# jenndrei/BayHunter

Hardware: AMD Instinct MI355X
Metric: forward-model+logL evals/sec (batched 10-layer models) (higher is better)
Workload: dtype f64

## Files before the change

bayhunter_amd/csrc/chain_kernel.hip:

```cpp
#include "../../include/bh_engine.h"
#include "bh_device.h"
#ifndef BH_CHAIN_ABSENT
#define BH_CHAIN_ABSENT 0
#endif
#ifndef BH_CHAIN_PRIORS
#define BH_CHAIN_PRIORS 0
#endif
#ifndef BH_CHAIN_RECORD
#define BH_CHAIN_RECORD 0
#endif
#if BH_CHAIN_RECORD
#include "../../include/bh_engine_chain_record.h"
#define BH_RECORD_KPARAM , bh_chain_record store, int due, int due_step
#else
#define BH_RECORD_KPARAM
#endif
#if BH_CHAIN_PRIORS
#include "../../include/bh_engine_sites_priors.h"
#define ST pr
#define BH_NLO(i) pr.nb[(i) * pr.stride]
#define BH_NHI(i) pr.nb[(2 * BH_MAX_TARGETS + (i)) * pr.stride]
#define BH_NOISE_FREE(i) (BH_NLO(i) != BH_NHI(i) && ((absent >> ((i) >> 1)) & 1u) == 0u)
#define BH_PRIOR_OK (!pr.bad)
#define BH_SITE_PARAM , unsigned absent, const Prior &pr
#define BH_SITE_ARG(c) , (absent_of != nullptr ? (unsigned)absent_of[c] : 0u), pr
#define BH_SITE_KPARAM , const uint8_t *absent_of, const bh_chain_prior *priors, int NP, const int32_t *prior_of
#define BH_ACCEPT_KPARAM , const bh_chain_prior *priors, int NP, const int32_t *prior_of
#elif BH_CHAIN_ABSENT
#include "../../include/bh_engine_sites_missing.h"
#define ST cfg
#define BH_NLO(i) cfg.noise_lo[i]
#define BH_NHI(i) cfg.noise_hi[i]
#define BH_NOISE_FREE(i) (cfg.noise_lo[i] != cfg.noise_hi[i] && ((absent >> ((i) >> 1)) & 1u) == 0u)
#define BH_PRIOR_OK true
#define BH_SITE_PARAM , unsigned absent
#define BH_SITE_ARG(c) , (unsigned)absent_of[c]
#define BH_SITE_KPARAM , const uint8_t *absent_of
#else
#define ST cfg
#define BH_NLO(i) cfg.noise_lo[i]
#define BH_NHI(i) cfg.noise_hi[i]
#define BH_NOISE_FREE(i) (cfg.noise_lo[i] != cfg.noise_hi[i])
#define BH_PRIOR_OK true
#define BH_SITE_PARAM
#define BH_SITE_ARG(c)
#define BH_SITE_KPARAM
#define BH_ACCEPT_KPARAM
#endif

namespace {

struct Philox {
    uint32_t k0, k1;
    __device__ void round(uint32_t c[4])
    {
        const uint32_t M0 = 0xD2511F53u, M1 = 0xCD9E8D57u;
        const uint64_t p0 = (uint64_t)M0 * c[0], p1 = (uint64_t)M1 * c[2];
        const uint32_t hi0 = (uint32_t)(p0 >> 32), lo0 = (uint32_t)p0, hi1 = (uint32_t)(p1 >> 32), lo1 = (uint32_t)p1;
        const uint32_t n0 = hi1 ^ c[1] ^ k0, n1 = lo1, n2 = hi0 ^ c[3] ^ k1, n3 = lo0;
        c[0] = n0; c[1] = n1; c[2] = n2; c[3] = n3;
        k0 += 0x9E3779B9u;
        k1 += 0xBB67AE85u;
    }
    __device__ void gen(uint64_t seed, uint32_t a, uint32_t b, uint32_t cc, uint32_t out[4])
    {
        k0 = (uint32_t)seed;
        k1 = (uint32_t)(seed >> 32);
        uint32_t c[4] = {a, b, cc, 0u};
        for (int i = 0; i < 10; ++i) round(c);
        out[0] = c[0]; out[1] = c[1]; out[2] = c[2]; out[3] = c[3];
    }
};

__device__ __forceinline__ double u01(uint32_t hi, uint32_t lo)
{
    return (double)((((uint64_t)hi << 32) | lo) >> 11) * (1.0 / 9007199254740992.0);
}

#if !BH_CHAIN_RECORD
struct Draws {
    double u_move, u_index, u_z, u_accept, u_noise, normal;
};

__device__ Draws get_draws(const bh_chain_config &cfg, const bh_chain_state &S, int c, int C, int iiter, int k)
{
    Draws d;
    if (S.inject != nullptr) {
        const double *in = S.inject + (size_t)k * 6 * C;
        d.u_move = in[0 * (size_t)C + c]; d.u_index = in[1 * (size_t)C + c];
        d.u_z = in[2 * (size_t)C + c]; d.u_accept = in[3 * (size_t)C + c];
        d.u_noise = in[4 * (size_t)C + c]; d.normal = in[5 * (size_t)C + c];
        return d;
    }
    Philox ph;
    uint32_t r[4], q[4], t[4], n[4];
    const uint32_t gc = (uint32_t)(cfg.chain_offset + (int64_t)c);
    ph.gen(cfg.seed, gc, (uint32_t)iiter, 0u, r);
    ph.gen(cfg.seed, gc, (uint32_t)iiter, 1u, q);
    ph.gen(cfg.seed, gc, (uint32_t)iiter, 2u, t);
    ph.gen(cfg.seed, gc, (uint32_t)iiter, 3u, n);
    d.u_move = u01(r[0], r[1]); d.u_index = u01(r[2], r[3]);
    d.u_z = u01(q[0], q[1]); d.u_accept = u01(q[2], q[3]);
    d.u_noise = u01(t[0], t[1]);
    const double a = 1.0 - u01(n[0], n[1]);
    const double bq = u01(n[2], n[3]);
    d.normal = sqrt(-2.0 * log(a)) * cospi(2.0 * bq);
    return d;
}
#endif

#if !BH_CHAIN_ABSENT
__device__ double get_accept_draw(const bh_chain_config &cfg, const bh_chain_state &S, int c, int C, int iiter, int k)
{
    if (S.inject != nullptr) return S.inject[(size_t)k * 6 * C + 3 * (size_t)C + c];
    Philox ph;
    uint32_t q[4];
    ph.gen(cfg.seed, (uint32_t)(cfg.chain_offset + (int64_t)c), (uint32_t)iiter, 1u, q);
    return u01(q[2], q[3]);
}
#endif

enum { MV_VS = 0, MV_Z = 1, MV_BIRTH = 2, MV_DEATH = 3, MV_NOISE = 4, MV_VPVS = 5 };
__device__ __forceinline__ int par_index(int mv) { return mv <= 1 ? mv : (mv <= 3 ? 2 : mv - 1); }

struct Params {
    int n;
    double vpvs;
    double *vs, *z, *noise, *h;
};
#if BH_CHAIN_PRIORS
struct Prior {
    int layermin, layermax;
    double vsmin, vsmax, zmin, zmax, thickmin, lvz, hvz, vpvsmin, vpvsmax, mantle_vs, mantle_vpvs;
    const double *nb;
    int stride;
    bool bad;
};
__device__ __forceinline__ void fetch_prior(Prior &pr, const bh_chain_prior *priors, int NP, int k, double *nb, int stride, int first,
                                            int step)
{
    pr.nb = nb;
    pr.stride = stride;
    pr.bad = k < 0 || k >= NP;
    if (pr.bad) {
        pr.layermin = pr.layermax = 0;
        pr.vsmin = pr.vsmax = pr.zmin = pr.zmax = pr.thickmin = pr.vpvsmin = pr.vpvsmax = pr.mantle_vpvs = 0.0;
        pr.lvz = pr.hvz = pr.mantle_vs = -1.0;
        for (int i = first; i < 4 * BH_MAX_TARGETS; i += step) nb[i * stride] = 0.0;
        return;
    }
    const bh_chain_prior *__restrict__ r = priors + k;
    pr.layermin = r->layermin; pr.layermax = r->layermax;
    pr.vsmin = r->vsmin; pr.vsmax = r->vsmax; pr.zmin = r->zmin; pr.zmax = r->zmax;
    pr.thickmin = r->thickmin; pr.lvz = r->lvz; pr.hvz = r->hvz;
    pr.vpvsmin = r->vpvsmin; pr.vpvsmax = r->vpvsmax; pr.mantle_vs = r->mantle_vs; pr.mantle_vpvs = r->mantle_vpvs;
    for (int i = first; i < 4 * BH_MAX_TARGETS; i += step)
        nb[i * stride] = i < 2 * BH_MAX_TARGETS ? r->noise_lo[i] : r->noise_hi[i - 2 * BH_MAX_TARGETS];
}
struct AcceptPrior {
    double vsmin, vsmax, acc_lo, acc_hi;
};
#endif
__host__ __device__ inline int node_rec_doubles(int nt, int ML) { return 3 + 2 * nt + 3 * (ML + 1); }

#if !BH_CHAIN_RECORD
__device__ void load_base(const bh_chain_state &S, int C, size_t ldp, int nt, int ML, int c, int from_node, Params &P,
                          const double *lds_from = nullptr)
{
    if (from_node >= 0 && lds_from != nullptr) {
        const double *__restrict__ src = lds_from;
        double *__restrict__ pn = P.noise, *__restrict__ pv = P.vs, *__restrict__ pz = P.z;
        P.n = (int)src[0];
        P.vpvs = src[2];
        for (int i = 0; i < 2 * nt; ++i) pn[i] = src[3 + i];
        const double *__restrict__ fv = src + 3 + 2 * nt, *__restrict__ fz = fv + (ML + 1);
        const int n = P.n;
#pragma unroll 4
        for (int i = 0; i < n; ++i) {
            pv[i] = fv[i];
            pz[i] = fz[i];
        }
        return;
    }
    if (from_node < 0) {
        P.n = S.n[c];
        for (int i = 0; i < P.n; ++i) {
            P.vs[i] = S.vs[(size_t)i * C + c];
            P.z[i] = S.z[(size_t)i * C + c];
        }
        P.vpvs = S.vpvs[c];
        for (int i = 0; i < 2 * nt; ++i) P.noise[i] = S.noise[(size_t)i * C + c];
    } else {
        const size_t col = (size_t)from_node * C + c;
        P.n = S.pn[col];
        for (int i = 0; i < P.n; ++i) {
            P.vs[i] = S.pvs[(size_t)i * ldp + col];
            P.z[i] = S.pz[(size_t)i * ldp + col];
        }
        P.vpvs = S.pvpvs[col];
        for (int i = 0; i < 2 * nt; ++i) P.noise[i] = S.pnoise[col * 2 * nt + i];
    }
}

__device__ __forceinline__ void layer_thicknesses(const Params &P, double *h_)
{
    const double *__restrict__ z = P.z;
    double *__restrict__ h = h_;
    const int n = P.n;
    double prev = 0.0, zi = n >= 1 ? z[0] : 0.0;
#pragma unroll 4
    for (int i = 0; i + 1 < n; ++i) {
        const double zn = z[i + 1];
        const double zd = (zi + zn) / 2.;
        h[i] = zd - prev;
        prev = zd;
        zi = zn;
    }
    if (n >= 1) h[n - 1] = 0.0;
}

__device__ __forceinline__ int nearest_nucleus(const double *__restrict__ z, int n, double zb)
{
    int near = 0;
    double best = fabs(z[0] - zb);
#pragma unroll 4
    for (int i = 1; i < n; ++i) {
        const double di = fabs(z[i] - zb);
        if (di < best) {
            best = di;
            near = i;
        }
    }
    return near;
}

__device__ __forceinline__ void propose_node(const bh_chain_config &cfg, const bh_chain_state &S, int C, size_t ldp, int c, int iiter,
                                             int from_node, int node, Params &P, const double *lds_from, bool *valid_out, const Draws &d BH_SITE_PARAM)
{
    const int ML = cfg.maxlayers, nt = cfg.nt;
    int nnoise = 0;
    for (int i = 0; i < 2 * nt; ++i) nnoise += BH_NOISE_FREE(i);
    const bool vpvs_free = ST.vpvsmin != ST.vpvsmax;
    const bool early = (double)iiter < (-(double)cfg.iter_burnin + (double)cfg.iterations * 0.01);
    int moves[6], nm = 0;
    moves[nm++] = MV_VS;
    moves[nm++] = MV_Z;
    if (!early) {
        moves[nm++] = MV_BIRTH;
        moves[nm++] = MV_DEATH;
    }
    if (nnoise > 0) moves[nm++] = MV_NOISE;
    if (vpvs_free) moves[nm++] = MV_VPVS;
    int mi = (int)(d.u_move * nm);
    if (mi >= nm) mi = nm - 1;
    const int mv = moves[mi];

    load_base(S, C, ldp, nt, ML, c, from_node, P, lds_from);
    double *vs = P.vs, *z = P.z, *noise = P.noise;
    int n = P.n;
    double vpvs = P.vpvs;
    double dvs2 = 0.0;
    bool valid = BH_PRIOR_OK;
    if (mv == MV_VS) {
        int ind = (int)(d.u_index * n);
        if (ind >= n) ind = n - 1;
        vs[ind] = vs[ind] + d.normal * S.propdist[0 * (size_t)C + c];
    } else if (mv == MV_Z) {
        int ind = (int)(d.u_index * n);
        if (ind >= n) ind = n - 1;
        z[ind] = z[ind] + d.normal * S.propdist[1 * (size_t)C + c];
    } else if (mv == MV_BIRTH) {
        const double zb = ST.zmin + d.u_z * (ST.zmax - ST.zmin);
        const int near = nearest_nucleus(z, n, zb);
        const double vb = vs[near] + d.normal * S.propdist[2 * (size_t)C + c];
        dvs2 = (vb - vs[near]) * (vb - vs[near]);
        if (n >= ML) valid = false;
        else {
            vs[n] = vb;
            z[n] = zb;
            n += 1;
        }
    } else if (mv == MV_DEATH) {
        int ind = (int)(d.u_index * n);
        if (ind >= n) ind = n - 1;
        const double zb = z[ind], vb = vs[ind];
        for (int i = ind; i + 1 < n; ++i) {
            vs[i] = vs[i + 1];
            z[i] = z[i + 1];
        }
        n -= 1;
        if (n < 1) valid = false;
        else {
            const int near = nearest_nucleus(z, n, zb);
            dvs2 = (vs[near] - vb) * (vs[near] - vb);
        }
    } else if (mv == MV_NOISE) {
        int pick = (int)(d.u_noise * nnoise);
        if (pick >= nnoise) pick = nnoise - 1;
        int idx = 0;
        for (int i = 0, seen = 0; i < 2 * nt; ++i)
            if (BH_NOISE_FREE(i)) {
                if (seen == pick) idx = i;
                ++seen;
            }
        noise[idx] = noise[idx] + d.normal * S.propdist[3 * (size_t)C + c];
        for (int i = 0; i < 2 * nt; ++i)
            if (BH_NOISE_FREE(i) && (noise[i] < BH_NLO(i) || noise[i] > BH_NHI(i))) valid = false;
    } else {
        vpvs = vpvs + d.normal * S.propdist[4 * (size_t)C + c];
        if (vpvs < ST.vpvsmin || vpvs > ST.vpvsmax) valid = false;
    }
    double ztop = n > 0 ? z[0] : 0.0;
    for (int i = 1; i < n; ++i) {
        const double zi = z[i];
        if (!(ztop > zi)) {
            ztop = zi;
            continue;
        }
        const double vi = vs[i];
        int j = i - 1;
        while (j >= 0 && z[j] > zi) {
            z[j + 1] = z[j];
            vs[j + 1] = vs[j];
            --j;
        }
        z[j + 1] = zi;
        vs[j + 1] = vi;
    }
    P.n = n;
    P.vpvs = vpvs;
    double *h = P.h;
    layer_thicknesses(P, h);
    if (valid && (mv <= MV_DEATH)) {
        const int layermodel = n - 1;
        if (!(layermodel >= ST.layermin && layermodel <= ST.layermax)) valid = false;
        const double *__restrict__ rh = h, *__restrict__ rv = vs;
        double zc = 0.0, vi = n > 0 ? rv[0] : 0.0;
        bool ok = true;
#pragma unroll 4
        for (int i = 0; i < n; ++i) {
            const double hi = rh[i];
            const double vn = (i + 1 < n) ? rv[i + 1] : 0.0;
            if (i < n - 1 && hi < ST.thickmin) ok = false;
            if (vi < ST.vsmin || vi > ST.vsmax) ok = false;
            zc += hi;
            if (zc < ST.zmin || zc > ST.zmax) ok = false;
            if (i + 1 < n) {
                if (ST.lvz >= 0.0 && !(vn - vi * (1 - ST.lvz) > 0)) ok = false;
                if (ST.hvz >= 0.0 && !(vi * (1 + ST.hvz) - vn > 0)) ok = false;
            }
            vi = vn;
        }
        valid = valid && ok;
    }
    const size_t col = (size_t)node * C + c;
    S.move[col] = mv;
    S.valid[col] = valid ? 1 : 0;
    S.dvs2[col] = dvs2;
    if (!valid) {
        load_base(S, C, ldp, nt, ML, c, from_node, P, lds_from);
        layer_thicknesses(P, h);
        n = P.n;
        vpvs = P.vpvs;
    }
    P.n = n;
    P.vpvs = vpvs;
    *valid_out = valid;
    S.pn[col] = n;
    S.pvpvs[col] = vpvs;
    for (int i = 0; i < 2 * nt; ++i) S.pnoise[col * 2 * nt + i] = noise[i];
    {
        const double *__restrict__ rv = vs, *__restrict__ rz = z, *__restrict__ rh = h;
        bool deep = false;
#pragma unroll 4
        for (int i = 0; i < n; ++i) {
            const double vi = rv[i], zi = rz[i], hi = rh[i];
            if (ST.mantle_vs > 0.0 && vi >= ST.mantle_vs) deep = true;
            S.pvs[(size_t)i * ldp + col] = vi;
            S.pz[(size_t)i * ldp + col] = zi;
            S.lay_h[(size_t)i * ldp + col] = hi;
            S.lay_vs[(size_t)i * ldp + col] = vi;
            const double vpi = vi * (deep ? ST.mantle_vpvs : vpvs);
            S.lay_vp[(size_t)i * ldp + col] = vpi;
            if (S.lay_rho != nullptr) S.lay_rho[(size_t)i * ldp + col] = vpi * 0.32 + 0.77;
        }
    }
    S.lay_n[col] = n;
}

__global__ void chain_propose_kernel(bh_chain_config cfg, bh_chain_state S, int C, int iiter BH_SITE_KPARAM)
{
    const int c = blockIdx.x * blockDim.x + threadIdx.x;
    if (c >= C) return;
    double vs[BH_CHAIN_MAXLAYERS + 1], z[BH_CHAIN_MAXLAYERS + 1], h[BH_CHAIN_MAXLAYERS + 1], noise[2 * BH_MAX_TARGETS];
    Params P;
    P.vs = vs; P.z = z; P.h = h; P.noise = noise;
#if BH_CHAIN_PRIORS
    __shared__ double nb[4 * BH_MAX_TARGETS * 64];
    Prior pr;
    fetch_prior(pr, priors, NP, prior_of[c], nb + threadIdx.x, 64, 0, 1);
#endif
    bool valid;
    propose_node(cfg, S, C, (size_t)C, c, iiter, -1, 0, P, nullptr, &valid, get_draws(cfg, S, c, C, iiter, 0) BH_SITE_ARG(c));
}

__global__ __launch_bounds__(64) void chain_propose_window_kernel(bh_chain_config cfg, bh_chain_state S, int C, size_t ldp,
                                                                   int iiter, int depth BH_SITE_KPARAM)
{
    extern __shared__ __align__(16) double tree[];
    const int T = 1 << (depth - 1);
    const int per_wg = 64 / T;
    const int N = (1 << depth) - 1;
    const int slot = (int)threadIdx.x / T;
    const int c = blockIdx.x * per_wg + slot;
    const int p = (int)threadIdx.x % T;
    const int nt = cfg.nt, ML = cfg.maxlayers;
    const int RS = node_rec_doubles(nt, ML) | 1;
    double *mine = tree + (size_t)slot * N * RS;
#if BH_CHAIN_PRIORS
    double *nbw = tree + (size_t)per_wg * N * RS;
    Prior pr;
    {
        fetch_prior(pr, priors, NP, c < C ? prior_of[c] : -1, nbw + slot, per_wg, p, T);
        __builtin_amdgcn_fence(__ATOMIC_RELEASE, "wavefront");
        __builtin_amdgcn_wave_barrier();
        __builtin_amdgcn_fence(__ATOMIC_ACQUIRE, "wavefront");
    }
#endif
    Draws mydraws = {0.0, 0.0, 0.0, 0.0, 0.0, 0.0};
    if (c < C && p < depth) mydraws = get_draws(cfg, S, c, C, iiter + p, p);
    for (int k = 0; k < depth; ++k) {
        const int srcl = slot * T + k;
        Draws d;
        d.u_move = __shfl(mydraws.u_move, srcl); d.u_index = __shfl(mydraws.u_index, srcl);
        d.u_z = __shfl(mydraws.u_z, srcl); d.u_accept = __shfl(mydraws.u_accept, srcl);
        d.u_noise = __shfl(mydraws.u_noise, srcl); d.normal = __shfl(mydraws.normal, srcl);
        if (c < C && p < (1 << k)) {
            const int node = (1 << k) - 1 + p;
            int from = -1;
            for (int j = node; j > 0; j = (j - 1) >> 1) {
                const int parent = (j - 1) >> 1;
                if ((j & 1) == 0 && mine[(size_t)parent * RS + 1] != 0.0) {
                    from = parent;
                    break;
                }
            }
            double *rec = mine + (size_t)node * RS;
            Params P;
            P.noise = rec + 3;
            P.vs = rec + 3 + 2 * nt;
            P.z = P.vs + (ML + 1);
            P.h = P.z + (ML + 1);
            bool valid;
            propose_node(cfg, S, C, ldp, c, iiter + k, from, node, P, from >= 0 ? mine + (size_t)from * RS : nullptr, &valid, d BH_SITE_ARG(c));
            rec[0] = (double)P.n;
            rec[1] = valid ? 1.0 : 0.0;
            rec[2] = P.vpvs;
        }
        __builtin_amdgcn_fence(__ATOMIC_RELEASE, "wavefront");
        __builtin_amdgcn_wave_barrier();
        __builtin_amdgcn_fence(__ATOMIC_ACQUIRE, "wavefront");
    }
}
#endif

#if !BH_CHAIN_ABSENT && !BH_CHAIN_RECORD
__global__ void chain_accept_kernel(bh_chain_config cfg, bh_chain_state S, int C, size_t ldp, int iiter, int depth,
                                    const double *logL, const double *misfits BH_ACCEPT_KPARAM)
{
    const int c = blockIdx.x * blockDim.x + threadIdx.x;
    if (c >= C) return;
#if BH_CHAIN_PRIORS
    const int rec = prior_of[c];
    if (rec < 0 || rec >= NP) return;
    const AcceptPrior pr = {priors[rec].vsmin, priors[rec].vsmax, priors[rec].acc_lo, priors[rec].acc_hi};
#endif
    const int nt = cfg.nt;
    int node = 0, last = -1;
    double cur = S.like[c];
    const double beta = S.beta ? S.beta[c] : 1.0;
    for (int k = 0; k < depth; ++k) {
        const size_t col = (size_t)node * C + c;
        bool accepted = false;
        if (S.valid[col]) {
            const double u_accept = get_accept_draw(cfg, S, c, C, iiter + k, k);
            const int mv = S.move[col];
            const int pi = par_index(mv);
            S.proposed[pi * (size_t)C + c] += 1.0;
            const double like = logL[col];
            const double dl = (S.beta ? beta * (like - cur) : like - cur);
            double alpha;
            if (mv == MV_BIRTH || mv == MV_DEATH) {
                const double theta = S.propdist[2 * (size_t)C + c];
                const double dv = ST.vsmax - ST.vsmin;
                const double Bt = S.dvs2[col] / (2. * (theta * theta));
                if (mv == MV_BIRTH) alpha = log((theta * sqrt(2 * M_PI)) / dv) + Bt + dl;
                else alpha = log(dv / (theta * sqrt(2 * M_PI))) - Bt + dl;
            } else {
                alpha = dl;
            }
            if (log(u_accept) < alpha) {
                accepted = true;
                last = node;
                cur = like;
                S.accepted[pi * (size_t)C + c] += 1.0;
                S.naccepted[c] += 1;
            }
            if ((iiter + k) % 1000 == 0) {
                bool all = true;
                for (int i = 0; i < 5; ++i) all = all && (S.proposed[i * (size_t)C + c] != 0.0);
                if (all)
                    for (int i = 0; i < 5; ++i) {
                        const double rate = S.accepted[i * (size_t)C + c] / S.proposed[i * (size_t)C + c] * 100;
                        double pd = S.propdist[i * (size_t)C + c];
                        if (rate < ST.acc_lo) {
                            pd = pd * 0.95;
                            if (pd < 0.001) pd = 0.001;
                        } else if (rate > ST.acc_hi) {
                            pd = pd * 1.05;
                        }
                        S.propdist[i * (size_t)C + c] = pd;
                    }
            }
        }
        node = 2 * node + (accepted ? 2 : 1);
    }
    if (last >= 0) {
        const size_t col = (size_t)last * C + c;
        const int n = S.pn[col];
        S.n[c] = n;
        for (int i = 0; i < n; ++i) {
            S.vs[(size_t)i * C + c] = S.pvs[(size_t)i * ldp + col];
            S.z[(size_t)i * C + c] = S.pz[(size_t)i * ldp + col];
        }
        for (int i = n; i < cfg.maxlayers; ++i) {
            S.vs[(size_t)i * C + c] = 0.0;
            S.z[(size_t)i * C + c] = 0.0;
        }
        S.vpvs[c] = S.pvpvs[col];
        for (int i = 0; i < 2 * nt; ++i) S.noise[(size_t)i * C + c] = S.pnoise[col * 2 * nt + i];
        S.like[c] = cur;
        for (int i = 0; i <= nt; ++i) S.misfits[(size_t)i * C + c] = misfits[col * (nt + 1) + i];
    }
}
// ... 120 lines not shown
    if (lane < 5) {
        S.proposed[lane * (size_t)C + c] = prop;
        S.accepted[lane * (size_t)C + c] = acc;
    }
    if (lane == 0) S.naccepted[c] = nacc;
    if (last >= 0) {
        const size_t col = (size_t)last * C + c;
        const int n = S.pn[col];
        for (int i = lane; i < cfg.maxlayers; i += 64) {
            S.vs[(size_t)i * C + c] = i < n ? S.pvs[(size_t)i * ldp + col] : 0.0;
            S.z[(size_t)i * C + c] = i < n ? S.pz[(size_t)i * ldp + col] : 0.0;
        }
        for (int i = lane; i < 2 * nt; i += 64) S.noise[(size_t)i * C + c] = S.pnoise[col * 2 * nt + i];
        for (int i = lane; i <= nt; i += 64) S.misfits[(size_t)i * C + c] = misfits[col * (nt + 1) + i];
        if (lane == 0) {
            S.n[c] = n;
            S.vpvs[c] = S.pvpvs[col];
            S.like[c] = cur;
        }
    }
}

#endif

}

extern "C" {

#if BH_CHAIN_RECORD
#if BH_CHAIN_PRIORS
int bh_chain_accept_window_priors_record(void *stream, const bh_chain_config *cfg, const bh_chain_state *state, int C, int iiter,
                                         int depth, ptrdiff_t ld, const double *logL, const double *misfits,
                                         const bh_chain_prior *priors, int P, const int32_t *prior_of, const bh_chain_record *rec)
#else
int bh_chain_accept_window_record(void *stream, const bh_chain_config *cfg, const bh_chain_state *state, int C, int iiter,
                                  int depth, ptrdiff_t ld, const double *logL, const double *misfits, const bh_chain_record *rec)
#endif
{
    if (!cfg || !state || C < 0 || !logL || !misfits) return BH_EINVAL;
    if (cfg->maxlayers < 0 || cfg->maxlayers > BH_CHAIN_MAXLAYERS || cfg->nt < 0 || cfg->nt > BH_MAX_TARGETS) return BH_EINVAL;
    if (depth < 1 || depth > BH_CHAIN_MAXDEPTH || ld < (ptrdiff_t)C * ((1 << depth) - 1)) return BH_EINVAL;
#if BH_CHAIN_PRIORS
    if (!priors || !prior_of || P < 1) return BH_EINVAL;
#endif
    for (int k = 0; k + 1 < depth; ++k)
        if ((iiter + k) % 1000 == 0) return BH_EINVAL;
    if (!rec || !rec->models || !rec->likes || !rec->vpvs || !rec->misfits || !rec->noise) return BH_EINVAL;
    if (rec->thinning < 1 || rec->row0 < 0) return BH_EINVAL;
    const int64_t res = (((int64_t)iiter % rec->thinning) + rec->thinning) % rec->thinning;
    const int64_t first = res == 0 ? 0 : rec->thinning - res;
    const int64_t m = first >= depth ? 0 : 1 + ((int64_t)depth - 1 - first) / rec->thinning;
    if (rec->row0 > rec->rows - m) return BH_EINVAL;
    if (C == 0) return BH_OK;
    const int due = (int)(first < depth ? first : depth);
    const int due_step = (int)(rec->thinning <= BH_CHAIN_MAXDEPTH ? rec->thinning : BH_CHAIN_MAXDEPTH + 1);
#if BH_CHAIN_PRIORS
    hipLaunchKernelGGL(chain_accept_window_kernel, dim3(C), dim3(64), 0, (hipStream_t)stream, *cfg, *state, C, (size_t)ld, iiter, depth,
                       logL, misfits, priors, P, prior_of, *rec, due, due_step);
#else
    hipLaunchKernelGGL(chain_accept_window_kernel, dim3(C), dim3(64), 0, (hipStream_t)stream, *cfg, *state, C, (size_t)ld, iiter, depth,
                       logL, misfits, *rec, due, due_step);
#endif
    return hipGetLastError() == hipSuccess ? BH_OK : BH_EHIP;
}

#elif BH_CHAIN_PRIORS
static int window_args_ok(const bh_chain_config *cfg, const bh_chain_state *state, int C, int iiter, int depth, ptrdiff_t ld,
                          const bh_chain_prior *priors, int P, const int32_t *prior_of)
{
    if (!cfg || !state || C < 0 || cfg->maxlayers > BH_CHAIN_MAXLAYERS || cfg->nt > BH_MAX_TARGETS) return 0;
    if (depth < 1 || depth > BH_CHAIN_MAXDEPTH || ld < (ptrdiff_t)C * ((1 << depth) - 1)) return 0;
    if (!priors || !prior_of || P < 1) return 0;
    for (int k = 0; k + 1 < depth; ++k)
        if ((iiter + k) % 1000 == 0) return 0;
    return 1;
}

int bh_chain_propose_window_priors(void *stream, const bh_chain_config *cfg, const bh_chain_state *state, int C, int iiter,
                                   int depth, ptrdiff_t ld, const bh_chain_prior *priors, int P, const int32_t *prior_of,
                                   const uint8_t *absent)
{
    if (!window_args_ok(cfg, state, C, iiter, depth, ld, priors, P, prior_of)) return BH_EINVAL;
    if (C == 0) return BH_OK;
    if (depth == 1 && ld == C) {
        hipLaunchKernelGGL(chain_propose_kernel, dim3((C + 63) / 64), dim3(64), 0, (hipStream_t)stream, *cfg, *state, C, iiter, absent,
                           priors, P, prior_of);
    } else {
        const int per_wg = 64 >> (depth - 1);
        const size_t lds = ((size_t)per_wg * ((1 << depth) - 1) * (node_rec_doubles(cfg->nt, cfg->maxlayers) | 1) +
                            (size_t)per_wg * 4 * BH_MAX_TARGETS) * sizeof(double);
        if (lds > 160 * 1024) return BH_EUNSUPPORTED;
        if (lds > 64 * 1024) {
            static std::atomic<unsigned long long> big{0};
            const void *k[1] = {reinterpret_cast<const void *>(chain_propose_window_kernel)};
            if (!bh_allow_big_lds(&big, k, 1, 160 * 1024)) return BH_EHIP;
        }
        hipLaunchKernelGGL(chain_propose_window_kernel, dim3((C + per_wg - 1) / per_wg), dim3(64), lds, (hipStream_t)stream, *cfg,
                           *state, C, (size_t)ld, iiter, depth, absent, priors, P, prior_of);
    }
    return hipGetLastError() == hipSuccess ? BH_OK : BH_EHIP;
}

int bh_chain_propose_priors(void *stream, const bh_chain_config *cfg, const bh_chain_state *state, int C, int iiter,
                            const bh_chain_prior *priors, int P, const int32_t *prior_of, const uint8_t *absent)
{
    return bh_chain_propose_window_priors(stream, cfg, state, C, iiter, 1, C, priors, P, prior_of, absent);
}

int bh_chain_accept_window_priors(void *stream, const bh_chain_config *cfg, const bh_chain_state *state, int C, int iiter,
                                  int depth, ptrdiff_t ld, const double *logL, const double *misfits,
                                  const bh_chain_prior *priors, int P, const int32_t *prior_of)
{
    if (!window_args_ok(cfg, state, C, iiter, depth, ld, priors, P, prior_of) || !logL || !misfits) return BH_EINVAL;
    if (C == 0) return BH_OK;
    if (depth > 1)
        hipLaunchKernelGGL(chain_accept_window_kernel, dim3(C), dim3(64), 0, (hipStream_t)stream, *cfg, *state, C, (size_t)ld, iiter, depth,
                           logL, misfits, priors, P, prior_of);
    else
        hipLaunchKernelGGL(chain_accept_kernel, dim3((C + 63) / 64), dim3(64), 0, (hipStream_t)stream, *cfg, *state, C, (size_t)ld,
                           iiter, depth, logL, misfits, priors, P, prior_of);
    return hipGetLastError() == hipSuccess ? BH_OK : BH_EHIP;
}

int bh_chain_accept_priors(void *stream, const bh_chain_config *cfg, const bh_chain_state *state, int C, int iiter,
                           const double *logL, const double *misfits, const bh_chain_prior *priors, int P,
                           const int32_t *prior_of)
{
    return bh_chain_accept_window_priors(stream, cfg, state, C, iiter, 1, C, logL, misfits, priors, P, prior_of);
}

#else

#if BH_CHAIN_ABSENT
int bh_chain_propose_window_sites(void *stream, const bh_chain_config *cfg, const bh_chain_state *state, int C, int iiter,
                                  int depth, ptrdiff_t ld, const uint8_t *absent)
#else
int bh_chain_propose_window(void *stream, const bh_chain_config *cfg, const bh_chain_state *state, int C, int iiter,
                            int depth, ptrdiff_t ld)
#endif
{
#if BH_CHAIN_ABSENT
    if (!absent) return BH_EINVAL;
#define BH_ABSENT_LAUNCH , absent
#else
#define BH_ABSENT_LAUNCH
#endif
    if (!cfg || !state || C < 0 || cfg->maxlayers > BH_CHAIN_MAXLAYERS || cfg->nt > BH_MAX_TARGETS) return BH_EINVAL;
    if (depth < 1 || depth > BH_CHAIN_MAXDEPTH || ld < (ptrdiff_t)C * ((1 << depth) - 1)) return BH_EINVAL;
    for (int k = 0; k + 1 < depth; ++k)
        if ((iiter + k) % 1000 == 0) return BH_EINVAL;
    if (C == 0) return BH_OK;
    if (depth == 1 && ld == C) {
        hipLaunchKernelGGL(chain_propose_kernel, dim3((C + 63) / 64), dim3(64), 0, (hipStream_t)stream, *cfg, *state, C, iiter BH_ABSENT_LAUNCH);
    } else {
        const int per_wg = 64 >> (depth - 1);
        const size_t lds = (size_t)per_wg * ((1 << depth) - 1) * (node_rec_doubles(cfg->nt, cfg->maxlayers) | 1) * sizeof(double);
        if (lds > 160 * 1024) return BH_EUNSUPPORTED;
        if (lds > 64 * 1024) {
            static std::atomic<unsigned long long> big{0};
            const void *k[1] = {reinterpret_cast<const void *>(chain_propose_window_kernel)};
            if (!bh_allow_big_lds(&big, k, 1, 160 * 1024)) return BH_EHIP;
        }
        hipLaunchKernelGGL(chain_propose_window_kernel, dim3((C + per_wg - 1) / per_wg), dim3(64), lds, (hipStream_t)stream, *cfg,
                           *state, C, (size_t)ld, iiter, depth BH_ABSENT_LAUNCH);
    }
    return hipGetLastError() == hipSuccess ? BH_OK : BH_EHIP;
}
#undef BH_ABSENT_LAUNCH

#if BH_CHAIN_ABSENT
int bh_chain_propose_sites(void *stream, const bh_chain_config *cfg, const bh_chain_state *state, int C, int iiter, const uint8_t *absent)
{
    return bh_chain_propose_window_sites(stream, cfg, state, C, iiter, 1, C, absent);
}
#else

int bh_chain_accept_window(void *stream, const bh_chain_config *cfg, const bh_chain_state *state, int C, int iiter, int depth,
                           ptrdiff_t ld, const double *logL, const double *misfits)
{
    if (!cfg || !state || C < 0 || !logL || !misfits) return BH_EINVAL;
    if (depth < 1 || depth > BH_CHAIN_MAXDEPTH || ld < (ptrdiff_t)C * ((1 << depth) - 1)) return BH_EINVAL;
    for (int k = 0; k + 1 < depth; ++k)
        if ((iiter + k) % 1000 == 0) return BH_EINVAL;
    if (C == 0) return BH_OK;
    if (depth > 1)
        hipLaunchKernelGGL(chain_accept_window_kernel, dim3(C), dim3(64), 0, (hipStream_t)stream, *cfg, *state, C, (size_t)ld, iiter, depth,
                           logL, misfits);
    else
        hipLaunchKernelGGL(chain_accept_kernel, dim3((C + 63) / 64), dim3(64), 0, (hipStream_t)stream, *cfg, *state, C, (size_t)ld,
                           iiter, depth, logL, misfits);
    return hipGetLastError() == hipSuccess ? BH_OK : BH_EHIP;
}

int bh_chain_propose(void *stream, const bh_chain_config *cfg, const bh_chain_state *state, int C, int iiter)
{
    return bh_chain_propose_window(stream, cfg, state, C, iiter, 1, C);
}

int bh_chain_accept(void *stream, const bh_chain_config *cfg, const bh_chain_state *state, int C, int iiter,
                    const double *logL, const double *misfits)
{
    return bh_chain_accept_window(stream, cfg, state, C, iiter, 1, C, logL, misfits);
}

#endif

#endif

}
```

Baseline: 6.170 million.

## Parallelise chain proposal across lanes per chain with one workgroup per chain

Rewrites the MCMC proposal kernel so each chain gets its own workgroup, and each tree node is handled by a group of lanes rather than one thread. Nearest-nucleus search, layer sorting (rank-based instead of insertion sort), thickness and constraint checks, and noise checks become lane-parallel with ballots and shuffles. The base model, draws and proposal widths are staged in LDS once, and moves are expressed as virtual edits over the parent record instead of copied arrays. The separate depth-1 kernel path is dropped. This trades more threads and LDS per chain, plus extra barriers, for less serial per-thread work.

New measurement: 6.150 million. About the same (-0.3%).

```diff
diff --git a/bayhunter_amd/csrc/chain_kernel.hip b/bayhunter_amd/csrc/chain_kernel.hip
--- a/bayhunter_amd/csrc/chain_kernel.hip
+++ b/bayhunter_amd/csrc/chain_kernel.hip
@@ -22,28 +22,30 @@
 #define BH_NHI(i) pr.nb[(2 * BH_MAX_TARGETS + (i)) * pr.stride]
 #define BH_NOISE_FREE(i) (BH_NLO(i) != BH_NHI(i) && ((absent >> ((i) >> 1)) & 1u) == 0u)
 #define BH_PRIOR_OK (!pr.bad)
-#define BH_SITE_PARAM , unsigned absent, const Prior &pr
-#define BH_SITE_ARG(c) , (absent_of != nullptr ? (unsigned)absent_of[c] : 0u), pr
+#define BH_SITE_PARAM , const Prior &pr
+#define BH_SITE_ARG , pr
+#define BH_ABSENT_OF(c) (absent_of != nullptr ? (unsigned)absent_of[c] : 0u)
 #define BH_SITE_KPARAM , const uint8_t *absent_of, const bh_chain_prior *priors, int NP, const int32_t *prior_of
 #define BH_ACCEPT_KPARAM , const bh_chain_prior *priors, int NP, const int32_t *prior_of
 #elif BH_CHAIN_ABSENT
 #include "../../include/bh_engine_sites_missing.h"
 #define ST cfg
-#define BH_NLO(i) cfg.noise_lo[i]
-#define BH_NHI(i) cfg.noise_hi[i]
-#define BH_NOISE_FREE(i) (cfg.noise_lo[i] != cfg.noise_hi[i] && ((absent >> ((i) >> 1)) & 1u) == 0u)
+#define BH_NLO(i) nb[i]
+#define BH_NHI(i) nb[2 * BH_MAX_TARGETS + (i)]
+#define BH_NOISE_FREE(i) (BH_NLO(i) != BH_NHI(i) && ((absent >> ((i) >> 1)) & 1u) == 0u)
 #define BH_PRIOR_OK true
-#define BH_SITE_PARAM , unsigned absent
-#define BH_SITE_ARG(c) , (unsigned)absent_of[c]
+#define BH_SITE_PARAM , const double *nb
+#define BH_SITE_ARG , nb
+#define BH_ABSENT_OF(c) ((unsigned)absent_of[c])
 #define BH_SITE_KPARAM , const uint8_t *absent_of
 #else
 #define ST cfg
-#define BH_NLO(i) cfg.noise_lo[i]
-#define BH_NHI(i) cfg.noise_hi[i]
-#define BH_NOISE_FREE(i) (cfg.noise_lo[i] != cfg.noise_hi[i])
+#define BH_NLO(i) nb[i]
+#define BH_NHI(i) nb[2 * BH_MAX_TARGETS + (i)]
+#define BH_NOISE_FREE(i) (BH_NLO(i) != BH_NHI(i))
 #define BH_PRIOR_OK true
-#define BH_SITE_PARAM
-#define BH_SITE_ARG(c)
+#define BH_SITE_PARAM , const double *nb
+#define BH_SITE_ARG , nb
 #define BH_SITE_KPARAM
 #define BH_ACCEPT_KPARAM
 #endif
@@ -123,11 +125,6 @@
 enum { MV_VS = 0, MV_Z = 1, MV_BIRTH = 2, MV_DEATH = 3, MV_NOISE = 4, MV_VPVS = 5 };
 __device__ __forceinline__ int par_index(int mv) { return mv <= 1 ? mv : (mv <= 3 ? 2 : mv - 1); }
 
-struct Params {
-    int n;
-    double vpvs;
-    double *vs, *z, *noise, *h;
-};
 #if BH_CHAIN_PRIORS
 struct Prior {
     int layermin, layermax;
@@ -162,220 +159,277 @@
 };
 #endif
 __host__ __device__ inline int node_rec_doubles(int nt, int ML) { return 3 + 2 * nt + 3 * (ML + 1); }
+#ifndef BH_PROPOSE_LANES
+#define BH_PROPOSE_LANES 32
+#endif
+#ifndef BH_PROPOSE_MAXTHREADS
+#define BH_PROPOSE_MAXTHREADS 512
+#endif
+__host__ __device__ inline int propose_threads(int depth)
+{
+    const int t = BH_PROPOSE_LANES << (depth - 1);
+    return t < 64 ? 64 : (t > BH_PROPOSE_MAXTHREADS ? BH_PROPOSE_MAXTHREADS : t);
+}
+enum { PROPOSE_HDR = 6 * BH_CHAIN_MAXDEPTH + 5 + 1 };
+__host__ __device__ inline size_t propose_lds_doubles(int nt, int ML, int depth)
+{
+    return ((size_t)1 << depth) * (size_t)(node_rec_doubles(nt, ML) | 1) + PROPOSE_HDR + 4 * BH_MAX_TARGETS + (((size_t)1 << depth) + 1) / 2;
+}
 
 #if !BH_CHAIN_RECORD
-__device__ void load_base(const bh_chain_state &S, int C, size_t ldp, int nt, int ML, int c, int from_node, Params &P,
-                          const double *lds_from = nullptr)
-{
-    if (from_node >= 0 && lds_from != nullptr) {
-        const double *__restrict__ src = lds_from;
-        double *__restrict__ pn = P.noise, *__restrict__ pv = P.vs, *__restrict__ pz = P.z;
-        P.n = (int)src[0];
-        P.vpvs = src[2];
-        for (int i = 0; i < 2 * nt; ++i) pn[i] = src[3 + i];
-        const double *__restrict__ fv = src + 3 + 2 * nt, *__restrict__ fz = fv + (ML + 1);
-        const int n = P.n;
-#pragma unroll 4
-        for (int i = 0; i < n; ++i) {
-            pv[i] = fv[i];
-            pz[i] = fz[i];
-        }
-        return;
-    }
-    if (from_node < 0) {
-        P.n = S.n[c];
-        for (int i = 0; i < P.n; ++i) {
-            P.vs[i] = S.vs[(size_t)i * C + c];
-            P.z[i] = S.z[(size_t)i * C + c];
-        }
-        P.vpvs = S.vpvs[c];
-        for (int i = 0; i < 2 * nt; ++i) P.noise[i] = S.noise[(size_t)i * C + c];
-    } else {
-        const size_t col = (size_t)from_node * C + c;
-        P.n = S.pn[col];
-        for (int i = 0; i < P.n; ++i) {
-            P.vs[i] = S.pvs[(size_t)i * ldp + col];
-            P.z[i] = S.pz[(size_t)i * ldp + col];
-        }
-        P.vpvs = S.pvpvs[col];
-        for (int i = 0; i < 2 * nt; ++i) P.noise[i] = S.pnoise[col * 2 * nt + i];
-    }
-}
-
-__device__ __forceinline__ void layer_thicknesses(const Params &P, double *h_)
-{
-    const double *__restrict__ z = P.z;
-    double *__restrict__ h = h_;
-    const int n = P.n;
-    double prev = 0.0, zi = n >= 1 ? z[0] : 0.0;
-#pragma unroll 4
-    for (int i = 0; i + 1 < n; ++i) {
-        const double zn = z[i + 1];
-        const double zd = (zi + zn) / 2.;
-        h[i] = zd - prev;
-        prev = zd;
-        zi = zn;
-    }
-    if (n >= 1) h[n - 1] = 0.0;
-}
-
-__device__ __forceinline__ int nearest_nucleus(const double *__restrict__ z, int n, double zb)
-{
-    int near = 0;
-    double best = fabs(z[0] - zb);
-#pragma unroll 4
-    for (int i = 1; i < n; ++i) {
-        const double di = fabs(z[i] - zb);
-        if (di < best) {
-            best = di;
-            near = i;
-        }
-    }
-    return near;
+struct Lanes {
+    int g, W, first;
+    unsigned long long mask;
+};
+__device__ __forceinline__ unsigned long long group_ballot(const Lanes &G, bool p) { return (__ballot(p) >> G.first) & G.mask; }
+__device__ __forceinline__ void group_sync()
+{
+    __builtin_amdgcn_fence(__ATOMIC_RELEASE, "wavefront");
+    __builtin_amdgcn_wave_barrier();
+    __builtin_amdgcn_fence(__ATOMIC_ACQUIRE, "wavefront");
+}
+
+struct Moved {
+    const double *sv, *sz;
+    int del, rv, rz;
+    double newv, newz;
+    __device__ __forceinline__ double z(int j) const
+    {
+        const double v = sz[j + (j >= del ? 1 : 0)];
+        return j == rz ? newz : v;
+    }
+    __device__ __forceinline__ double vs(int j) const
+    {
+        const double v = sv[j + (j >= del ? 1 : 0)];
+        return j == rv ? newv : v;
+    }
+};
+
+__device__ __forceinline__ int nearest_nucleus(const Lanes &G, const Moved &M, int n, double zb)
+{
+    double best = __builtin_huge_val();
+    int near = 0x7fffffff;
+    for (int i0 = 0; i0 < n; i0 += G.W) {
+        const int i = i0 + G.g;
+        if (i < n) {
+            const double di = fabs(M.z(i) - zb);
+            if (i == 0 || di < best) {
+                best = di;
+                near = i;
+            }
+        }
+    }
+    for (int off = G.W >> 1; off >= 1; off >>= 1) {
+        const double bo = __shfl_xor(best, off);
+        const int no = __shfl_xor(near, off);
+        if (bo < best || (bo == best && no < near)) {
+            best = bo;
+            near = no;
+        }
+    }
+    near = __shfl(near, G.first);
+    return near < 0 ? 0 : (near < n ? near : (n > 0 ? n - 1 : 0));
+}
+
+__device__ __forceinline__ bool layers_of(const Lanes &G, int n, const double *ov, const double *oz, double *oh, bool check,
+                                          double thickmin, double vsmin, double vsmax, double lvz, double hvz)
+{
+    bool anybad = false;
+    for (int i0 = 0; i0 < n; i0 += G.W) {
+        const int i = i0 + G.g;
+        bool bad = false;
+        if (i < n) {
+            const double zi = oz[i];
+            const double prev = i > 0 ? (oz[i - 1] + zi) / 2. : 0.0;
+            double hi = 0.0;
+            if (i + 1 < n) {
+                const double zd = (zi + oz[i + 1]) / 2.;
+                hi = zd - prev;
+            }
+            oh[i] = hi;
+            if (check) {
+                const double vi = ov[i];
+                if (i < n - 1 && hi < thickmin) bad = true;
+                if (vi < vsmin || vi > vsmax) bad = true;
+                if (i + 1 < n) {
+                    const double vn = ov[i + 1];
+                    if (lvz >= 0.0 && !(vn - vi * (1 - lvz) > 0)) bad = true;
+                    if (hvz >= 0.0 && !(vi * (1 + hvz) - vn > 0)) bad = true;
+                }
+            }
+        }
+        if (check && group_ballot(G, bad) != 0ull) anybad = true;
+    }
+    return anybad;
 }
 
 __device__ __forceinline__ void propose_node(const bh_chain_config &cfg, const bh_chain_state &S, int C, size_t ldp, int c, int iiter,
-                                             int from_node, int node, Params &P, const double *lds_from, bool *valid_out, const Draws &d BH_SITE_PARAM)
-{
-    const int ML = cfg.maxlayers, nt = cfg.nt;
-    int nnoise = 0;
-    for (int i = 0; i < 2 * nt; ++i) nnoise += BH_NOISE_FREE(i);
+                                             int node, const double *src, double *rec, const Lanes &G, const Draws &d, const double *pd,
+                                             unsigned nfree BH_SITE_PARAM)
+{
+    const int ML = cfg.maxlayers, nt = cfg.nt, g = G.g, W = G.W;
+    const int nnoise = __popc(nfree);
     const bool vpvs_free = ST.vpvsmin != ST.vpvsmax;
     const bool early = (double)iiter < (-(double)cfg.iter_burnin + (double)cfg.iterations * 0.01);
-    int moves[6], nm = 0;
-    moves[nm++] = MV_VS;
-    moves[nm++] = MV_Z;
-    if (!early) {
-        moves[nm++] = MV_BIRTH;
-        moves[nm++] = MV_DEATH;
-    }
-    if (nnoise > 0) moves[nm++] = MV_NOISE;
-    if (vpvs_free) moves[nm++] = MV_VPVS;
+    const int nm = 2 + (early ? 0 : 2) + (nnoise > 0 ? 1 : 0) + (vpvs_free ? 1 : 0);
     int mi = (int)(d.u_move * nm);
     if (mi >= nm) mi = nm - 1;
-    const int mv = moves[mi];
-
-    load_base(S, C, ldp, nt, ML, c, from_node, P, lds_from);
-    double *vs = P.vs, *z = P.z, *noise = P.noise;
-    int n = P.n;
-    double vpvs = P.vpvs;
-    double dvs2 = 0.0;
+    int mv;
+    if (mi < 2) mv = mi;
+    else if (!early && mi < 4) mv = mi;
+    else mv = (nnoise > 0 && mi == (early ? 2 : 4)) ? MV_NOISE : MV_VPVS;
+
+    const double *sn = src + 3, *sv = src + 3 + 2 * nt, *sz = sv + (ML + 1);
+    double *on = rec + 3, *ov = rec + 3 + 2 * nt, *oz = ov + (ML + 1), *oh = oz + (ML + 1);
+    const int n0 = (int)src[0];
+    const double vpvs0 = src[2];
+    int n = n0, noise_at = -1;
+    double vpvs = vpvs0, dvs2 = 0.0;
     bool valid = BH_PRIOR_OK;
-    if (mv == MV_VS) {
-        int ind = (int)(d.u_index * n);
-        if (ind >= n) ind = n - 1;
-        vs[ind] = vs[ind] + d.normal * S.propdist[0 * (size_t)C + c];
-    } else if (mv == MV_Z) {
-        int ind = (int)(d.u_index * n);
-        if (ind >= n) ind = n - 1;
-        z[ind] = z[ind] + d.normal * S.propdist[1 * (size_t)C + c];
-    } else if (mv == MV_BIRTH) {
-        const double zb = ST.zmin + d.u_z * (ST.zmax - ST.zmin);
-        const int near = nearest_nucleus(z, n, zb);
-        const double vb = vs[near] + d.normal * S.propdist[2 * (size_t)C + c];
-        dvs2 = (vb - vs[near]) * (vb - vs[near]);
-        if (n >= ML) valid = false;
+    Moved M = {sv, sz, 0x7fffffff, -1, -1, 0.0, 0.0};
+    if (mv <= MV_Z) {
+        int ind = (int)(d.u_index * n0);
+        if (ind >= n0) ind = n0 - 1;
+        if (ind < 0) ind = 0;
+        if (mv == MV_VS) {
+            M.newv = sv[ind] + d.normal * pd[0];
+            M.rv = ind;
+        } else {
+            M.newz = sz[ind] + d.normal * pd[1];
+            M.rz = ind;
+        }
+    } else if (mv <= MV_DEATH) {
+        double zb, vb = 0.0;
+        int among = n0;
+        if (mv == MV_BIRTH) zb = ST.zmin + d.u_z * (ST.zmax - ST.zmin);
         else {
-            vs[n] = vb;
-            z[n] = zb;
-            n += 1;
-        }
-    } else if (mv == MV_DEATH) {
-        int ind = (int)(d.u_index * n);
-        if (ind >= n) ind = n - 1;
-        const double zb = z[ind], vb = vs[ind];
-        for (int i = ind; i + 1 < n; ++i) {
-            vs[i] = vs[i + 1];
-            z[i] = z[i + 1];
-        }
-        n -= 1;
-        if (n < 1) valid = false;
-        else {
-            const int near = nearest_nucleus(z, n, zb);
-            dvs2 = (vs[near] - vb) * (vs[near] - vb);
+            int ind = (int)(d.u_index * n0);
+            if (ind >= n0) ind = n0 - 1;
+            if (ind < 0) ind = 0;
+            zb = sz[ind];
+            vb = sv[ind];
+            M.del = ind;
+            n = n0 - 1;
+            if (n < 1) {
+                valid = false;
+                n = 0;
+            }
+            among = n;
+        }
+        if (among >= 1) {
+            const int near = nearest_nucleus(G, M, among, zb);
+            const double vn = M.vs(near);
+            if (mv == MV_BIRTH) {
+                vb = vn + d.normal * pd[2];
+                dvs2 = (vb - vn) * (vb - vn);
+            } else {
+                dvs2 = (vn - vb) * (vn - vb);
+            }
+        }
+        if (mv == MV_BIRTH) {
+            if (n0 >= ML) valid = false;
+            else {
+                M.rv = M.rz = n0;
+                M.newv = vb;
+                M.newz = zb;
+                n = n0 + 1;
+            }
         }
     } else if (mv == MV_NOISE) {
         int pick = (int)(d.u_noise * nnoise);
         if (pick >= nnoise) pick = nnoise - 1;
-        int idx = 0;
-        for (int i = 0, seen = 0; i < 2 * nt; ++i)
-            if (BH_NOISE_FREE(i)) {
-                if (seen == pick) idx = i;
-                ++seen;
-            }
-        noise[idx] = noise[idx] + d.normal * S.propdist[3 * (size_t)C + c];
-        for (int i = 0; i < 2 * nt; ++i)
-            if (BH_NOISE_FREE(i) && (noise[i] < BH_NLO(i) || noise[i] > BH_NHI(i))) valid = false;
+        unsigned b = nfree;
+        for (int k = 0; k < pick; ++k) b &= b - 1u;
+        noise_at = b != 0u ? __ffs(b) - 1 : 0;
     } else {
-        vpvs = vpvs + d.normal * S.propdist[4 * (size_t)C + c];
+        vpvs = vpvs0 + d.normal * pd[4];
         if (vpvs < ST.vpvsmin || vpvs > ST.vpvsmax) valid = false;
     }
-    double ztop = n > 0 ? z[0] : 0.0;
-    for (int i = 1; i < n; ++i) {
-        const double zi = z[i];
-        if (!(ztop > zi)) {
-            ztop = zi;
-            continue;
-        }
-        const double vi = vs[i];
-        int j = i - 1;
-        while (j >= 0 && z[j] > zi) {
-            z[j + 1] = z[j];
-            vs[j + 1] = vs[j];
-            --j;
-        }
-        z[j + 1] = zi;
-        vs[j + 1] = vi;
-    }
-    P.n = n;
-    P.vpvs = vpvs;
-    double *h = P.h;
-    layer_thicknesses(P, h);
-    if (valid && (mv <= MV_DEATH)) {
+    for (int i0 = 0; i0 < 2 * nt; i0 += W) {
+        const int i = i0 + g;
+        bool bad = false;
+        if (i < 2 * nt) {
+            double v = sn[i];
+            if (i == noise_at) v = v + d.normal * pd[3];
+            on[i] = v;
+            if (mv == MV_NOISE && ((nfree >> i) & 1u) != 0u && (v < BH_NLO(i) || v > BH_NHI(i))) bad = true;
+        }
+        if (group_ballot(G, bad) != 0ull) valid = false;
+    }
+    for (int i0 = 0; i0 < n; i0 += W) {
+        const int i = i0 + g;
+        if (i < n) oh[i] = M.z(i);
+    }
+    group_sync();
+    for (int i0 = 0; i0 < n; i0 += W) {
+        const int i = i0 + g;
+        if (i < n) {
+            const double zi = oh[i], vi = M.vs(i);
+            int r = 0;
+#pragma unroll 8
+            for (int j = 0; j < n; ++j) {
+                const double zj = oh[j];
+                r += (zj < zi || (zj == zi && j < i)) ? 1 : 0;
+            }
+            oz[r] = zi;
+            ov[r] = vi;
+        }
+    }
+    group_sync();
+    const bool check = valid && mv <= MV_DEATH;
+    if (check) {
         const int layermodel = n - 1;
         if (!(layermodel >= ST.layermin && layermodel <= ST.layermax)) valid = false;
-        const double *__restrict__ rh = h, *__restrict__ rv = vs;
-        double zc = 0.0, vi = n > 0 ? rv[0] : 0.0;
+    }
+    if (layers_of(G, n, ov, oz, oh, check, ST.thickmin, ST.vsmin, ST.vsmax, ST.lvz, ST.hvz)) valid = false;
+    group_sync();
+    if (check) {
+        double zc = 0.0;
         bool ok = true;
-#pragma unroll 4
+#pragma unroll 8
         for (int i = 0; i < n; ++i) {
-            const double hi = rh[i];
-            const double vn = (i + 1 < n) ? rv[i + 1] : 0.0;
-            if (i < n - 1 && hi < ST.thickmin) ok = false;
-            if (vi < ST.vsmin || vi > ST.vsmax) ok = false;
-            zc += hi;
+            zc += oh[i];
             if (zc < ST.zmin || zc > ST.zmax) ok = false;
-            if (i + 1 < n) {
-                if (ST.lvz >= 0.0 && !(vn - vi * (1 - ST.lvz) > 0)) ok = false;
-                if (ST.hvz >= 0.0 && !(vi * (1 + ST.hvz) - vn > 0)) ok = false;
-            }
-            vi = vn;
-        }
-        valid = valid && ok;
+        }
+        if (!ok) valid = false;
+    }
+    if (!valid) {
+        n = n0;
+        vpvs = vpvs0;
+        for (int i0 = 0; i0 < n; i0 += W) {
+            const int i = i0 + g;
+            if (i < n) {
+                oz[i] = sz[i];
+                ov[i] = sv[i];
+            }
+        }
+        for (int i = g; i < 2 * nt; i += W) on[i] = sn[i];
+        group_sync();
+        layers_of(G, n, ov, oz, oh, false, 0.0, 0.0, 0.0, 0.0, 0.0);
+        group_sync();
     }
     const size_t col = (size_t)node * C + c;
-    S.move[col] = mv;
-    S.valid[col] = valid ? 1 : 0;
-    S.dvs2[col] = dvs2;
-    if (!valid) {
-        load_base(S, C, ldp, nt, ML, c, from_node, P, lds_from);
-        layer_thicknesses(P, h);
-        n = P.n;
-        vpvs = P.vpvs;
-    }
-    P.n = n;
-    P.vpvs = vpvs;
-    *valid_out = valid;
-    S.pn[col] = n;
-    S.pvpvs[col] = vpvs;
-    for (int i = 0; i < 2 * nt; ++i) S.pnoise[col * 2 * nt + i] = noise[i];
-    {
-        const double *__restrict__ rv = vs, *__restrict__ rz = z, *__restrict__ rh = h;
-        bool deep = false;
-#pragma unroll 4
-        for (int i = 0; i < n; ++i) {
-            const double vi = rv[i], zi = rz[i], hi = rh[i];
-            if (ST.mantle_vs > 0.0 && vi >= ST.mantle_vs) deep = true;
+    if (g == 0) {
+        rec[0] = (double)n;
+        rec[1] = valid ? 1.0 : 0.0;
+        rec[2] = vpvs;
+        S.move[col] = mv;
+        S.valid[col] = valid ? 1 : 0;
+        S.dvs2[col] = dvs2;
+        S.pn[col] = n;
+        S.pvpvs[col] = vpvs;
+        S.lay_n[col] = n;
+    }
+    for (int i = g; i < 2 * nt; i += W) S.pnoise[col * 2 * nt + i] = on[i];
+    bool deep_before = false;
+    for (int i0 = 0; i0 < n; i0 += W) {
+        const int i = i0 + g;
+        double vi = 0.0;
+        if (i < n) vi = ov[i];
+        const unsigned long long m = group_ballot(G, i < n && ST.mantle_vs > 0.0 && vi >= ST.mantle_vs);
+        const bool deep = deep_before || (m & ((2ull << g) - 1ull)) != 0ull;
+        if (i < n) {
+            const double zi = oz[i], hi = oh[i];
             S.pvs[(size_t)i * ldp + col] = vi;
             S.pz[(size_t)i * ldp + col] = zi;
             S.lay_h[(size_t)i * ldp + col] = hi;
@@ -384,82 +438,82 @@
             S.lay_vp[(size_t)i * ldp + col] = vpi;
             if (S.lay_rho != nullptr) S.lay_rho[(size_t)i * ldp + col] = vpi * 0.32 + 0.77;
         }
-    }
-    S.lay_n[col] = n;
-}
-
-__global__ void chain_propose_kernel(bh_chain_config cfg, bh_chain_state S, int C, int iiter BH_SITE_KPARAM)
-{
-    const int c = blockIdx.x * blockDim.x + threadIdx.x;
-    if (c >= C) return;
-    double vs[BH_CHAIN_MAXLAYERS + 1], z[BH_CHAIN_MAXLAYERS + 1], h[BH_CHAIN_MAXLAYERS + 1], noise[2 * BH_MAX_TARGETS];
-    Params P;
-    P.vs = vs; P.z = z; P.h = h; P.noise = noise;
-#if BH_CHAIN_PRIORS
-    __shared__ double nb[4 * BH_MAX_TARGETS * 64];
-    Prior pr;
-    fetch_prior(pr, priors, NP, prior_of[c], nb + threadIdx.x, 64, 0, 1);
-#endif
-    bool valid;
-    propose_node(cfg, S, C, (size_t)C, c, iiter, -1, 0, P, nullptr, &valid, get_draws(cfg, S, c, C, iiter, 0) BH_SITE_ARG(c));
-}
-
-__global__ __launch_bounds__(64) void chain_propose_window_kernel(bh_chain_config cfg, bh_chain_state S, int C, size_t ldp,
-                                                                   int iiter, int depth BH_SITE_KPARAM)
+        deep_before = deep_before || m != 0ull;
+    }
+}
+
+__global__ __launch_bounds__(BH_PROPOSE_MAXTHREADS) void chain_propose_window_kernel(bh_chain_config cfg, bh_chain_state S, int C, size_t ldp,
+                                                                     int iiter, int depth BH_SITE_KPARAM)
 {
     extern __shared__ __align__(16) double tree[];
-    const int T = 1 << (depth - 1);
-    const int per_wg = 64 / T;
+    const int tid = (int)threadIdx.x, NT = (int)blockDim.x;
+    const int c = (int)blockIdx.x;
     const int N = (1 << depth) - 1;
-    const int slot = (int)threadIdx.x / T;
-    const int c = blockIdx.x * per_wg + slot;
-    const int p = (int)threadIdx.x % T;
     const int nt = cfg.nt, ML = cfg.maxlayers;
     const int RS = node_rec_doubles(nt, ML) | 1;
-    double *mine = tree + (size_t)slot * N * RS;
+    double *hdr = tree + (size_t)(N + 1) * RS;
+    double *pd = hdr + 6 * BH_CHAIN_MAXDEPTH;
 #if BH_CHAIN_PRIORS
-    double *nbw = tree + (size_t)per_wg * N * RS;
     Prior pr;
+    fetch_prior(pr, priors, NP, prior_of[c], hdr + PROPOSE_HDR, 1, tid, NT);
+#else
+    double *nb = hdr + PROPOSE_HDR;
+    for (int i = tid; i < 2 * BH_MAX_TARGETS; i += NT) {
+        nb[i] = cfg.noise_lo[i];
+        nb[2 * BH_MAX_TARGETS + i] = cfg.noise_hi[i];
+    }
+#endif
     {
-        fetch_prior(pr, priors, NP, c < C ? prior_of[c] : -1, nbw + slot, per_wg, p, T);
-        __builtin_amdgcn_fence(__ATOMIC_RELEASE, "wavefront");
-        __builtin_amdgcn_wave_barrier();
-        __builtin_amdgcn_fence(__ATOMIC_ACQUIRE, "wavefront");
-    }
-#endif
-    Draws mydraws = {0.0, 0.0, 0.0, 0.0, 0.0, 0.0};
-    if (c < C && p < depth) mydraws = get_draws(cfg, S, c, C, iiter + p, p);
+        int n = S.n[c];
+        n = n < 0 ? 0 : (n > ML ? ML : n);
+        double *r0v = tree + 3 + 2 * nt, *r0z = r0v + (ML + 1);
+        for (int i = tid; i < n; i += NT) {
+            r0v[i] = S.vs[(size_t)i * C + c];
+            r0z[i] = S.z[(size_t)i * C + c];
+        }
+        for (int i = tid; i < 2 * nt; i += NT) tree[3 + i] = S.noise[(size_t)i * C + c];
+        if (tid == 0) {
+            tree[0] = (double)n;
+            tree[1] = 1.0;
+            tree[2] = S.vpvs[c];
+        }
+        if (tid < 5) pd[tid] = S.propdist[(size_t)tid * C + c];
+    }
+    if (tid < depth) {
+        const Draws w = get_draws(cfg, S, c, C, iiter + tid, tid);
+        double *o = hdr + 6 * tid;
+        o[0] = w.u_move; o[1] = w.u_index; o[2] = w.u_z; o[3] = w.u_accept; o[4] = w.u_noise; o[5] = w.normal;
+    }
+    __syncthreads();
+#if BH_CHAIN_PRIORS || BH_CHAIN_ABSENT
+    const unsigned absent = BH_ABSENT_OF(c);
+#endif
+    const unsigned nfree = (unsigned)__ballot((tid & 63) < 2 * nt && BH_NOISE_FREE(tid & 63));
+    int *base_of = reinterpret_cast<int *>(hdr + PROPOSE_HDR + 4 * BH_MAX_TARGETS);
+    int lg = 6;
+    while ((1 << lg) < NT) ++lg;
     for (int k = 0; k < depth; ++k) {
-        const int srcl = slot * T + k;
-        Draws d;
-        d.u_move = __shfl(mydraws.u_move, srcl); d.u_index = __shfl(mydraws.u_index, srcl);
-        d.u_z = __shfl(mydraws.u_z, srcl); d.u_accept = __shfl(mydraws.u_accept, srcl);
-        d.u_noise = __shfl(mydraws.u_noise, srcl); d.normal = __shfl(mydraws.normal, srcl);
-        if (c < C && p < (1 << k)) {
+        const int per = NT >> k;
+        const int p = tid >> (lg - k), g = tid & (per - 1);
+        if (g < 64) {
+            Lanes G;
+            G.g = g;
+            G.W = per < 64 ? per : 64;
+            G.first = (tid & 63) & ~(G.W - 1);
+            G.mask = G.W == 64 ? ~0ull : ((1ull << G.W) - 1ull);
+            const double *dk = hdr + 6 * k;
+            const Draws d = {dk[0], dk[1], dk[2], dk[3], dk[4], dk[5]};
             const int node = (1 << k) - 1 + p;
             int from = -1;
-            for (int j = node; j > 0; j = (j - 1) >> 1) {
-                const int parent = (j - 1) >> 1;
-                if ((j & 1) == 0 && mine[(size_t)parent * RS + 1] != 0.0) {
-                    from = parent;
-                    break;
-                }
-            }
-            double *rec = mine + (size_t)node * RS;
-            Params P;
-            P.noise = rec + 3;
-            P.vs = rec + 3 + 2 * nt;
-            P.z = P.vs + (ML + 1);
-            P.h = P.z + (ML + 1);
-            bool valid;
-            propose_node(cfg, S, C, ldp, c, iiter + k, from, node, P, from >= 0 ? mine + (size_t)from * RS : nullptr, &valid, d BH_SITE_ARG(c));
-            rec[0] = (double)P.n;
-            rec[1] = valid ? 1.0 : 0.0;
-            rec[2] = P.vpvs;
-        }
-        __builtin_amdgcn_fence(__ATOMIC_RELEASE, "wavefront");
-        __builtin_amdgcn_wave_barrier();
-        __builtin_amdgcn_fence(__ATOMIC_ACQUIRE, "wavefront");
+            if (node > 0) {
+                const int parent = (node - 1) >> 1;
+                from = ((node & 1) == 0 && tree[(size_t)(parent + 1) * RS + 1] != 0.0) ? parent : base_of[parent];
+            }
+            if (g == 0) base_of[node] = from;
+            propose_node(cfg, S, C, ldp, c, iiter + k, node, tree + (size_t)(from + 1) * RS, tree + (size_t)(node + 1) * RS, G, d, pd,
+                         nfree BH_SITE_ARG);
+        }
+        __syncthreads();
     }
 }
 #endif
@@ -746,20 +800,15 @@
 {
     if (!window_args_ok(cfg, state, C, iiter, depth, ld, priors, P, prior_of)) return BH_EINVAL;
     if (C == 0) return BH_OK;
-    if (depth == 1 && ld == C) {
-        hipLaunchKernelGGL(chain_propose_kernel, dim3((C + 63) / 64), dim3(64), 0, (hipStream_t)stream, *cfg, *state, C, iiter, absent,
-                           priors, P, prior_of);
-    } else {
-        const int per_wg = 64 >> (depth - 1);
-        const size_t lds = ((size_t)per_wg * ((1 << depth) - 1) * (node_rec_doubles(cfg->nt, cfg->maxlayers) | 1) +
-                            (size_t)per_wg * 4 * BH_MAX_TARGETS) * sizeof(double);
+    {
+        const size_t lds = propose_lds_doubles(cfg->nt, cfg->maxlayers, depth) * sizeof(double);
         if (lds > 160 * 1024) return BH_EUNSUPPORTED;
         if (lds > 64 * 1024) {
             static std::atomic<unsigned long long> big{0};
             const void *k[1] = {reinterpret_cast<const void *>(chain_propose_window_kernel)};
             if (!bh_allow_big_lds(&big, k, 1, 160 * 1024)) return BH_EHIP;
         }
-        hipLaunchKernelGGL(chain_propose_window_kernel, dim3((C + per_wg - 1) / per_wg), dim3(64), lds, (hipStream_t)stream, *cfg,
+        hipLaunchKernelGGL(chain_propose_window_kernel, dim3(C), dim3(propose_threads(depth)), lds, (hipStream_t)stream, *cfg,
                            *state, C, (size_t)ld, iiter, depth, absent, priors, P, prior_of);
     }
     return hipGetLastError() == hipSuccess ? BH_OK : BH_EHIP;
@@ -814,18 +863,15 @@
     for (int k = 0; k + 1 < depth; ++k)
         if ((iiter + k) % 1000 == 0) return BH_EINVAL;
     if (C == 0) return BH_OK;
-    if (depth == 1 && ld == C) {
-        hipLaunchKernelGGL(chain_propose_kernel, dim3((C + 63) / 64), dim3(64), 0, (hipStream_t)stream, *cfg, *state, C, iiter BH_ABSENT_LAUNCH);
-    } else {
-        const int per_wg = 64 >> (depth - 1);
-        const size_t lds = (size_t)per_wg * ((1 << depth) - 1) * (node_rec_doubles(cfg->nt, cfg->maxlayers) | 1) * sizeof(double);
+    {
+        const size_t lds = propose_lds_doubles(cfg->nt, cfg->maxlayers, depth) * sizeof(double);
         if (lds > 160 * 1024) return BH_EUNSUPPORTED;
         if (lds > 64 * 1024) {
             static std::atomic<unsigned long long> big{0};
             const void *k[1] = {reinterpret_cast<const void *>(chain_propose_window_kernel)};
             if (!bh_allow_big_lds(&big, k, 1, 160 * 1024)) return BH_EHIP;
         }
-        hipLaunchKernelGGL(chain_propose_window_kernel, dim3((C + per_wg - 1) / per_wg), dim3(64), lds, (hipStream_t)stream, *cfg,
+        hipLaunchKernelGGL(chain_propose_window_kernel, dim3(C), dim3(propose_threads(depth)), lds, (hipStream_t)stream, *cfg,
                            *state, C, (size_t)ld, iiter, depth BH_ABSENT_LAUNCH);
     }
     return hipGetLastError() == hipSuccess ? BH_OK : BH_EHIP;
```
